# alexxx-db/dbx-distributed-pytorch-examples

Measured on AMD Instinct MI355X. Metric: images/sec (whole node) ResNet-50 ImageNet-1K at 1/2/4/8 MI355X; top-1 acc, higher is better.
Workload: dtype bf16; 1 GPU; model=resnet50 ImageNet-1K 224x224 1000 classes large-batch (global 8192 at 8 GPUs), global_batch=1024, per_gpu_batch=1024, parallelism=dp1, world_size_seen=1, backend=none, impl=native, optimizer=SGD momentum 0.9 nesterov=False wd 5e-5, memory_format=nhwc, graphs=True, ddp=none, kernels=dbx HIP (conv implicit-GEMM MFMA + fused BN/ReLU/pool/CE/SGD)

## Files before the change

### dbx_distributed_pytorch_examples_amd/csrc/nn_ops.hip

```cpp
#include "common.h"
#include "bn_fin.h"
#include "entry.h"

namespace dbx {

__device__ __forceinline__ void shard_sums(const double* stats, int nshard, int C, int c0, double& s_out,
                                           double& q_out, bool& active, int& c) {
  __shared__ double rs[8][33], rq[8][33];
  const int j = threadIdx.x & 7, k = threadIdx.x >> 3;
  c = c0 + j;
  double s = 0.0, q = 0.0;
  if (c < C) {
    for (int kk = k; kk < nshard; kk += 32) { s += stats[(size_t)kk * 2 * C + c]; q += stats[(size_t)kk * 2 * C + C + c]; }
  }
  rs[j][k] = s; rq[j][k] = q;
  __syncthreads();
  active = (k == 0) && (c < C);
  if (active) {
    double ss = 0.0, qq = 0.0;
    for (int t = 0; t < 32; ++t) { ss += rs[j][t]; qq += rq[j][t]; }
    s_out = ss; q_out = qq;
  }
}

// ... 345 lines not shown
    if constexpr (KF > 0) {
      u32x4 win[KF * KF];
      bool ok[KF * KF];
#pragma unroll
      for (int r = 0; r < KF; ++r)
#pragma unroll
        for (int ss = 0; ss < KF; ++ss) {
          const int hh = p * stride - pad + r, w = q * stride - pad + ss;
          const bool v = (unsigned)hh < (unsigned)H && (unsigned)w < (unsigned)W;
          ok[r * KF + ss] = v;
          win[r * KF + ss] = *reinterpret_cast<const u32x4*>(
              x + (((size_t)n * H + (v ? hh : 0)) * W + (v ? w : 0)) * C + c0);
        }
#pragma unroll
      for (int k = 0; k < KF * KF; ++k) {
        float f[8];
        unpack8(win[k], f);
#pragma unroll
        for (int j = 0; j < 8; ++j) {
          float v = f[j] * s[j] + h[j];
          if (relu) v = fmaxf(v, 0.f);
          if (ok[k] && v > best[j]) { best[j] = v; braw[j] = f[j]; bi[j] = (unsigned char)k; }
        }
      }
    }
    for (int r = 0; r < (KF > 0 ? 0 : K); ++r) {
      const int hh = p * stride - pad + r;
      if (hh < 0 || hh >= H) continue;
      for (int ss = 0; ss < K; ++ss) {
        const int w = q * stride - pad + ss;
        if (w < 0 || w >= W) continue;
        float f[8];
        unpack8(*reinterpret_cast<const u32x4*>(x + (((size_t)n * H + hh) * W + w) * C + c0), f);
#pragma unroll
        for (int j = 0; j < 8; ++j) {
          float v = f[j] * s[j] + h[j];
          if (relu) v = fmaxf(v, 0.f);
          if (v > best[j]) { best[j] = v; braw[j] = f[j]; bi[j] = (unsigned char)(r * K + ss); }
        }
      }
    }
    const size_t o = (size_t)pix * C + c0;
    *reinterpret_cast<u32x4*>(out + o) = pack8(best);
    *reinterpret_cast<uint2*>(arg + o) = *reinterpret_cast<uint2*>(bi);
    if (ymax) *reinterpret_cast<u32x4*>(ymax + o) = pack8(braw);
  }
}

__global__ void maxpool_bwd_kernel(const bf16* __restrict__ dout, const unsigned char* __restrict__ arg,
                                   bf16* __restrict__ dx, int N, int H, int W, int C, int P, int Q, int K,
                                   int stride, int pad) {
  const int cpt = C / 8;
  const long long total = (long long)N * H * W * cpt;
  for (long long i = (long long)blockIdx.x * blockDim.x + threadIdx.x; i < total; i += (long long)gridDim.x * blockDim.x) {
    const int cg = (int)(i % cpt);
    long long pix = i / cpt;
    const int w = (int)(pix % W); pix /= W;
    const int h = (int)(pix % H);
    const int n = (int)(pix / H);
    const int c0 = cg * 8;
    float acc[8] = {0, 0, 0, 0, 0, 0, 0, 0};
    const int p_lo = max(0, (h + pad - K + stride) / stride), p_hi = min(P - 1, (h + pad) / stride);
    const int q_lo = max(0, (w + pad - K + stride) / stride), q_hi = min(Q - 1, (w + pad) / stride);
    for (int p = p_lo; p <= p_hi; ++p) {
      const int r = h - (p * stride - pad);
      if (r < 0 || r >= K) continue;
      for (int q = q_lo; q <= q_hi; ++q) {
        const int s = w - (q * stride - pad);
        if (s < 0 || s >= K) continue;
        const size_t o = (((size_t)n * P + p) * Q + q) * C + c0;
        float g[8];
        unpack8(*reinterpret_cast<const u32x4*>(dout + o), g);
        const uint2 av = *reinterpret_cast<const uint2*>(arg + o);
        const unsigned char* a8 = reinterpret_cast<const unsigned char*>(&av);
        const unsigned char me = (unsigned char)(r * K + s);
#pragma unroll
        for (int j = 0; j < 8; ++j) acc[j] += (a8[j] == me) ? g[j] : 0.f;
      }
    }
    *reinterpret_cast<u32x4*>(dx + (((size_t)n * H + h) * W + w) * C + c0) = pack8(acc);
  }
}

template <bool APPLY>
__global__ __launch_bounds__(256) void pool_bn_bwd_kernel(const bf16* __restrict__ dpool,
                                                          const unsigned char* __restrict__ arg,
                                                          const bf16* __restrict__ y, const float* __restrict__ sc,
                                                          const float* __restrict__ sh, const float* __restrict__ c1,
                                                          const float* __restrict__ c2, const float* __restrict__ c3,
                                                          bf16* __restrict__ dy, double* __restrict__ stats, int nshard,
                                                          int N, int H, int W, int C, int P, int Q, int K, int stride,
                                                          int pad) {
  const int cpt = C >> 3;
  const int tid = threadIdx.x;
  const int c0 = (tid % cpt) * 8;
  float s_[8], h_[8], k1[8], k2[8], k3[8];
  load8f(sc + c0, s_);
  load8f(sh + c0, h_);
  load8f(c1 + c0, k1);
  load8f(c2 + c0, k2);
  if (APPLY) load8f(c3 + c0, k3);
  float as[8] = {0, 0, 0, 0, 0, 0, 0, 0}, aq[8] = {0, 0, 0, 0, 0, 0, 0, 0};
  const int rows = N * H, per_row = W * cpt;
  for (int row = blockIdx.x; row < rows; row += gridDim.x) {
    const int n = row / H, h = row - n * H;
    const int p_lo = max(0, (h + pad - K + stride) / stride), p_hi = min(P - 1, (h + pad) / stride);
    const int r_lo = h + pad - p_lo * stride;
    const bool p1 = p_hi >= p_lo, p2 = p_hi > p_lo;
    const int pc = p1 ? p_lo : 0;
    const int prow0 = (n * P + pc) * Q, prow1 = (n * P + (p2 ? p_lo + 1 : pc)) * Q;
    for (int i = tid; i < per_row; i += 256) {
      const int w = i / cpt;
      const int q_lo = max(0, (w + pad - K + stride) / stride);
      u32x4 gd[2][2];
      uint2 av[2][2];
      bool ok[2][2];
#pragma unroll
      for (int t = 0; t < 2; ++t) {
        const int q = q_lo + t;
        const int s = w + pad - q * stride;
        const bool vq = q < Q && s >= 0 && s < K;
        const int qq = vq ? q : 0;
#pragma unroll
        for (int u = 0; u < 2; ++u) {
          const int o = ((u ? prow1 : prow0) + qq) * C + c0;
          gd[u][t] = *reinterpret_cast<const u32x4*>(dpool + o);
          av[u][t] = *reinterpret_cast<const uint2*>(arg + o);
          ok[u][t] = vq && (u == 0 ? p1 : p2);
        }
      }
      const int e = (row * W + w) * C + c0;
      float yv[8];
      unpack8(*reinterpret_cast<const u32x4*>(y + e), yv);
      float g[8] = {0, 0, 0, 0, 0, 0, 0, 0};
#pragma unroll
      for (int u = 0; u < 2; ++u)
#pragma unroll
        for (int t = 0; t < 2; ++t) {
          const int r = r_lo - u * stride, s = w + pad - (q_lo + t) * stride;
          const unsigned me = (unsigned)(r * K + s);
          float gv[8];
          unpack8(gd[u][t], gv);
          const unsigned char* a8 = reinterpret_cast<const unsigned char*>(&av[u][t]);
#pragma unroll
          for (int j = 0; j < 8; ++j) g[j] += (ok[u][t] && a8[j] == me) ? gv[j] : 0.f;
        }
#pragma unroll
      for (int j = 0; j < 8; ++j) g[j] = (yv[j] * s_[j] + h_[j]) > 0.f ? g[j] : 0.f;
      if (APPLY) {
        float o[8];
#pragma unroll
        for (int j = 0; j < 8; ++j) o[j] = k1[j] * g[j] + k2[j] * yv[j] + k3[j];
        *reinterpret_cast<u32x4*>(dy + e) = pack8(o);
      } else {
#pragma unroll
        for (int j = 0; j < 8; ++j) { as[j] += g[j]; aq[j] += g[j] * (yv[j] - k1[j]) * k2[j]; }
      }
    }
  }
  if (!APPLY) {
    __shared__ float red[2][256 * 8];
#pragma unroll
    for (int j = 0; j < 8; ++j) { red[0][tid * 8 + j] = as[j]; red[1][tid * 8 + j] = aq[j]; }
    __syncthreads();
    double* st = stats + (size_t)(blockIdx.x % nshard) * 2 * C;
    for (int c = tid; c < C; c += 256) {
      const int gi = c / 8, j = c % 8;
      float ss = 0.f, qq = 0.f;
      for (int r = 0; r < 256 / cpt; ++r) { ss += red[0][(r * cpt + gi) * 8 + j]; qq += red[1][(r * cpt + gi) * 8 + j]; }
      atomicAdd(st + c, (double)ss);
      atomicAdd(st + C + c, (double)qq);
    }
  }
}

__global__ void avgpool_fwd_kernel(const bf16* __restrict__ x, bf16* __restrict__ out, int N, int HW, int C) {
  const int n = blockIdx.y;
  const int c0 = (blockIdx.x * blockDim.x + threadIdx.x) * 8;
  if (c0 >= C) return;
  float acc[8] = {0, 0, 0, 0, 0, 0, 0, 0};
  for (int i = 0; i < HW; ++i) {
    float f[8];
    unpack8(*reinterpret_cast<const u32x4*>(x + ((size_t)n * HW + i) * C + c0), f);
#pragma unroll
    for (int j = 0; j < 8; ++j) acc[j] += f[j];
  }
  const float inv = 1.f / HW;
#pragma unroll
  for (int j = 0; j < 8; ++j) acc[j] *= inv;
  *reinterpret_cast<u32x4*>(out + (size_t)n * C + c0) = pack8(acc);
}

__global__ void avgpool_bwd_kernel(const bf16* __restrict__ dout, bf16* __restrict__ dx, int N, int HW, int C) {
  const long long total = (long long)N * HW * C / 8;
  const float inv = 1.f / HW;
  for (long long i = (long long)blockIdx.x * blockDim.x + threadIdx.x; i < total; i += (long long)gridDim.x * blockDim.x) {
    const long long e = i * 8;
    const int c0 = (int)(e % C);
    const long long n = e / ((long long)HW * C);
    float f[8];
    unpack8(*reinterpret_cast<const u32x4*>(dout + n * C + c0), f);
#pragma unroll
    for (int j = 0; j < 8; ++j) f[j] *= inv;
    *reinterpret_cast<u32x4*>(dx + e) = pack8(f);
  }
}

template <typename T>
__global__ void softmax_ce_kernel(const T* __restrict__ logits, const long long* __restrict__ labels,
                                  T* __restrict__ dlogits, float* __restrict__ loss_out, double* stats,
                                  int B, int C, float smoothing, float gscale,
                                  const long long* __restrict__ labels2, const float* __restrict__ lam_ptr) {
  const int row = blockIdx.x;
  const T* x = logits + (size_t)row * C;
  const int tid = threadIdx.x;
  __shared__ float red[8];
  __shared__ int redi[8];
  float mx = -INFINITY;
  int amx = 0;
  for (int c = tid; c < C; c += 256) {
    const float v = (float)x[c];
    if (v > mx) { mx = v; amx = c; }
  }
  for (int o = 32; o > 0; o >>= 1) {
    const float om = __shfl_xor(mx, o, 64);
    const int oa = __shfl_xor(amx, o, 64);
    if (om > mx || (om == mx && oa < amx)) { mx = om; amx = oa; }
  }
  const int wid = tid >> 6, lane = tid & 63;
  if (lane == 0) { red[wid] = mx; redi[wid] = amx; }
  __syncthreads();
  if (tid == 0) {
    for (int w = 1; w < 4; ++w)
      if (red[w] > red[0] || (red[w] == red[0] && redi[w] < redi[0])) { red[0] = red[w]; redi[0] = redi[w]; }
  }
  __syncthreads();
  mx = red[0];
  amx = redi[0];
  __syncthreads();
  float se = 0.f, sx = 0.f;
  for (int c = tid; c < C; c += 256) {
    const float v = (float)x[c];
    se += __expf(v - mx);
    sx += v;
// ... 247 lines not shown
extern "C" int dbx_bn_apply(const bf16* y, const float* sc, const float* sh, const bf16* res, const float* rsc,
                            const float* rsh, bf16* out, long long n, int C, int res_mode, int relu,
                            unsigned char* mbits, hipStream_t st, const BnFin* fin, const BnFin* rfin) {
  if (n % C || C % 8 || C / 8 > 256) return -1;
  if (rfin && res_mode != 2) return -2;
  const long long M = n / C;
  const dim3 g(grid_for(M, 256 / (C / 8), (fin || rfin) ? fin_cap(C) : 4096)), b(256);
#define BA(R, A) hipLaunchKernelGGL((bn_apply_kernel<R, A>), g, b, 0, st, y, sc, sh, res, rsc, rsh, out, mbits, M, C, fin, rfin)
  if (res_mode == 0) { if (relu) BA(0, true); else BA(0, false); }
  else if (res_mode == 1) { if (relu) BA(1, true); else BA(1, false); }
  else { if (relu) BA(2, true); else BA(2, false); }
#undef BA
  RET_LAST;
}
extern "C" int dbx_bn_bwd_reduce(const bf16* dout, const bf16* mref, const bf16* y, const float* sc, const float* sh,
                                 const float* mean, const float* invstd, long long M, int C, double* stats,
                                 int nshard, int mask_mode, hipStream_t st) {
  if (C % 8 || C / 8 > 256) return -1;
  const int rpb = 256 / (C / 8);
  const dim3 g(grid_for(M, rpb, 2048)), b(256);
  if (mask_mode == 0) hipLaunchKernelGGL((bn_bwd_reduce_kernel<0>), g, b, 0, st, dout, mref, y, sc, sh, mean, invstd, M, C, stats, nshard);
  else if (mask_mode == 1) hipLaunchKernelGGL((bn_bwd_reduce_kernel<1>), g, b, 0, st, dout, mref, y, sc, sh, mean, invstd, M, C, stats, nshard);
  else hipLaunchKernelGGL((bn_bwd_reduce_kernel<2>), g, b, 0, st, dout, mref, y, sc, sh, mean, invstd, M, C, stats, nshard);
  RET_LAST;
}
extern "C" int dbx_bn_bwd_coeff(const double* stats, int nshard, int C, float count, const float* gamma,
                                const float* mean, const float* invstd, float* coeff, float* dgamma, float* dbeta,
                                int accumulate, hipStream_t st) {
  hipLaunchKernelGGL(bn_bwd_coeff_kernel, dim3((C + 7) / 8), dim3(256), 0, st, stats, nshard, C, count, gamma,
                     mean, invstd, coeff, dgamma, dbeta, accumulate);
  RET_LAST;
}
extern "C" int dbx_bn_bwd_apply(const bf16* dout, const bf16* mref, const bf16* y, const float* sc, const float* sh,
                                const float* coeff, bf16* dy, bf16* gout, long long n, int C, int mask_mode,
                                hipStream_t st, const BnFin* fin) {
  if (n % C || C % 8 || C / 8 > 256) return -1;
  const long long M = n / C;
  const dim3 g(grid_for(M, 256 / (C / 8), fin ? fin_cap(C) : 4096)), b(256);
#define BB(MK, WG) hipLaunchKernelGGL((bn_bwd_apply_kernel<MK, WG>), g, b, 0, st, dout, mref, y, sc, sh, coeff, dy, gout, M, C, fin)
  if (mask_mode == 0) { if (gout) BB(0, true); else BB(0, false); }
  else if (mask_mode == 1) { if (gout) BB(1, true); else BB(1, false); }
  else { if (gout) BB(2, true); else BB(2, false); }
#undef BB
  RET_LAST;
}
extern "C" int dbx_bn_bwd_apply2(const bf16* g, const bf16* y1, const float* c1, bf16* dy1, const bf16* y2,
                                 const float* c2, bf16* dy2, long long n, int C, hipStream_t st, const BnFin* fin1,
                                 const BnFin* fin2) {
  if (n % C || C % 8 || C / 8 > 256) return -1;
  const long long M = n / C;
  hipLaunchKernelGGL(bn_bwd_apply2_kernel, dim3(grid_for(M, 256 / (C / 8), (fin1 || fin2) ? fin_cap(C) : 4096)), dim3(256), 0, st, g, y1, c1, dy1,
                     y2, c2, dy2, M, C, fin1, fin2);
  RET_LAST;
}
extern "C" int dbx_maxpool_fwd(const bf16* x, const float* sc, const float* sh, bf16* out, unsigned char* arg,
                               bf16* ymax, int N, int H, int W, int C, int P, int Q, int K, int stride, int pad, int relu,
                               hipStream_t st, const BnFin* fin) {
  if (C % 8) return -1;
  if (C / 8 > 256) return -1;
  if (fin && !sc) return -2;
  const dim3 grid(grid_for((long long)N * P * Q, 256 / (C / 8), fin ? 1024 : 4096));
  if (K == 3 && (long long)N * P * Q < (1ll << 31))
    hipLaunchKernelGGL(maxpool_fwd_kernel<3>, grid, dim3(256), 0, st, x, sc, sh, out, arg, ymax, N, H, W, C, P, Q, K,
                       stride, pad, relu, fin);
  else
    hipLaunchKernelGGL(maxpool_fwd_kernel<0>, grid, dim3(256), 0, st, x, sc, sh, out, arg, ymax, N, H, W, C, P, Q, K,
                       stride, pad, relu, fin);
  RET_LAST;
}
extern "C" int dbx_maxpool_bwd(const bf16* dout, const unsigned char* arg, bf16* dx, int N, int H, int W, int C, int P,
                               int Q, int K, int stride, int pad, hipStream_t st) {
  if (C % 8) return -1;
  const long long total = (long long)N * H * W * (C / 8);
  hipLaunchKernelGGL(maxpool_bwd_kernel, dim3(grid_for(total)), dim3(256), 0, st, dout, arg, dx, N, H, W, C, P, Q, K,
                     stride, pad);
  RET_LAST;
}
extern "C" int dbx_pool_bn_bwd(const bf16* dpool, const unsigned char* arg, const bf16* y, const float* sc,
                               const float* sh, const float* c1, const float* c2, const float* c3, bf16* dy,
                               double* stats, int nshard, int N, int H, int W, int C, int P, int Q, int K, int stride,
                               int pad, int apply, hipStream_t st) {
  if (C % 8 || 256 % (C / 8) || (K + stride - 1) / stride > 2) return -1;
  if ((long long)N * H * W * C >= (1LL << 31) || (long long)N * P * Q * C >= (1LL << 31)) return -2;
  const dim3 g(grid_for((long long)N * H, 1, apply ? 8192 : 2048)), b(256);
  if (apply)
    hipLaunchKernelGGL((pool_bn_bwd_kernel<true>), g, b, 0, st, dpool, arg, y, sc, sh, c1, c2, c3, dy, stats, nshard,
                       N, H, W, C, P, Q, K, stride, pad);
  else
    hipLaunchKernelGGL((pool_bn_bwd_kernel<false>), g, b, 0, st, dpool, arg, y, sc, sh, c1, c2, c3, dy, stats, nshard,
                       N, H, W, C, P, Q, K, stride, pad);
  RET_LAST;
}
extern "C" int dbx_avgpool_fwd(const bf16* x, bf16* out, int N, int HW, int C, hipStream_t st) {
  if (C % 8) return -1;
  hipLaunchKernelGGL(avgpool_fwd_kernel, dim3((C / 8 + 63) / 64, N), dim3(64), 0, st, x, out, N, HW, C);
  RET_LAST;
}
extern "C" int dbx_avgpool_bwd(const bf16* dout, bf16* dx, int N, int HW, int C, hipStream_t st) {
  if (C % 8) return -1;
  hipLaunchKernelGGL(avgpool_bwd_kernel, dim3(grid_for((long long)N * HW * C / 8)), dim3(256), 0, st, dout, dx, N, HW, C);
  RET_LAST;
}
extern "C" int dbx_softmax_ce(const void* logits, int is_bf16, const long long* labels, void* dlogits, float* loss_out,
                              double* stats, int B, int C, float smoothing, float gscale, const long long* labels2,
                              const float* lam, hipStream_t st, int kind, float target_thresh, int sum_classes) {
  if (kind == 1) {
    if (B <= 0) return 0;
    if (!logits || !labels || C < 1 || (labels2 && !lam)) return -1;
    const dim3 grid((B + 3) / 4);
    if (is_bf16)
      hipLaunchKernelGGL(bce_logits_kernel<bf16>, grid, dim3(256), 0, st, (const bf16*)logits, labels, (bf16*)dlogits,
                         loss_out, stats, B, C, smoothing, gscale, labels2, lam, target_thresh, sum_classes);
    else
      hipLaunchKernelGGL(bce_logits_kernel<float>, grid, dim3(256), 0, st, (const float*)logits, labels,
                         (float*)dlogits, loss_out, stats, B, C, smoothing, gscale, labels2, lam, target_thresh,
                         sum_classes);
    RET_LAST;
  }
  if (kind != 0) return -1;
  if (is_bf16)
    hipLaunchKernelGGL(softmax_ce_kernel<bf16>, dim3(B), dim3(256), 0, st, (const bf16*)logits, labels, (bf16*)dlogits,
                       loss_out, stats, B, C, smoothing, gscale, labels2, lam);
  else
    hipLaunchKernelGGL(softmax_ce_kernel<float>, dim3(B), dim3(256), 0, st, (const float*)logits, labels,
                       (float*)dlogits, loss_out, stats, B, C, smoothing, gscale, labels2, lam);
  RET_LAST;
}
extern "C" int dbx_ce_eval(const void* logits, int is_bf16, const long long* labels, double* stats, int B, int C, int k,
                           const int* nvalid, float* loss_out, int* rank_out, hipStream_t st) {
  if (B <= 0) return 0;
  if (!logits || !labels || !stats || C < 1 || k < 1 || k > C) return -1;
  const dim3 grid((B + 3) / 4);
  if (is_bf16)
    hipLaunchKernelGGL(ce_eval_kernel<bf16>, grid, dim3(256), 0, st, (const bf16*)logits, labels, stats, B, C, k, nvalid,
                       loss_out, rank_out);
  else
    hipLaunchKernelGGL(ce_eval_kernel<float>, grid, dim3(256), 0, st, (const float*)logits, labels, stats, B, C, k,
                       nvalid, loss_out, rank_out);
  RET_LAST;
}
extern "C" int dbx_weight_prep(const float* master, bf16* wbuf, const void* desc_dev, int nlayers, hipStream_t st) {
  hipLaunchKernelGGL(weight_prep_kernel<float>, dim3(512, nlayers), dim3(256), 0, st, master, wbuf,
                     (const WDesc*)desc_dev, nlayers);
  RET_LAST;
}
extern "C" int dbx_weight_prep16(const bf16* src, bf16* wbuf, const void* desc_dev, int nlayers, hipStream_t st) {
  hipLaunchKernelGGL(weight_prep_kernel<bf16>, dim3(512, nlayers), dim3(256), 0, st, src, wbuf,
                     (const WDesc*)desc_dev, nlayers);
  RET_LAST;
}
extern "C" int dbx_cast_f32_bf16(const float* x, bf16* y, long long n, hipStream_t st) {
  hipLaunchKernelGGL(cast_f32_bf16_kernel, dim3(grid_for(n)), dim3(256), 0, st, x, y, n);
  RET_LAST;
}
```

### dbx_distributed_pytorch_examples_amd/engine/program.py

```python
from __future__ import annotations

import math
import os
from dataclasses import dataclass, field
from typing import Dict, List, Optional, Tuple

import torch
import torch.nn as nn

from ..engine_config import EngineConfig
from ..models.resnet import BasicBlock, Bottleneck, CifarBlock, CifarResNet18, ResNet
from ..ops import kernels as K

IMAGENET_MEAN = (0.485, 0.456, 0.406)
IMAGENET_STD = (0.229, 0.224, 0.225)


def _repoint(p: nn.Parameter, view: torch.Tensor) -> None:
    p.data = view
    if p.grad is not None and (p.grad.device != view.device or p.grad.shape != view.shape):
        p.grad = None
    elif p.grad is not None and p.grad.stride() != view.stride():
        g = torch.empty_strided(view.shape, view.stride(), dtype=p.grad.dtype, device=view.device)
        g.copy_(p.grad)
# ... 278 lines not shown
                    _repoint(cv.mod.weight, view)
                    cv.grad = self.grad[off:off + n].view(cv.OC, cv.R * cv.S * cv.IC)
                    self.param_ranges.append((cv.name + ".weight", off, n))
                elif kind in ("bn_w", "bn_b"):
                    bn: BNL = obj
                    mod = bn.mod
                    p = getattr(mod, attr)
                    flat = self.master[off:off + n]
                    flat.copy_(p.detach().to(dev, torch.float32))
                    _repoint(p, flat)
                    if kind == "bn_w":
                        bn.off_w, bn.gamma, bn.dgamma = off, flat, self.grad[off:off + n]
                        bn.gamma_t = flat
                    else:
                        bn.off_b, bn.beta, bn.dbeta = off, flat, self.grad[off:off + n]
                        bn.beta_t = flat
                    self.param_ranges.append((f"{bn.name}.{attr}", off, n))
                    mod.running_mean.data = mod.running_mean.data.to(dev, torch.float32)
                    mod.running_var.data = mod.running_var.data.to(dev, torch.float32)
                    if kind == "bn_w" and mod.num_batches_tracked is not None:
                        nbt_vals.append(int(mod.num_batches_tracked))
                        nbt_mods.append(mod)
                else:
                    p = getattr(self.fc, attr)
                    flat = self.master[off:off + n]
                    flat.copy_(p.detach().reshape(-1).to(dev, torch.float32))
                    view = flat.view(p.shape)
                    _repoint(p, view)
                    if attr == "weight":
                        self.fc_w_off, self.fc_w_grad = off, self.grad[off:off + n].view(p.shape)
                    else:
                        self.fc_b_off, self.fc_b_grad = off, self.grad[off:off + n]
                    self.param_ranges.append((f"fc.{attr}", off, n))
        self.param16 = torch.zeros(total, device=dev, dtype=torch.bfloat16) if self._want_param16 else None
        self.nbt = torch.tensor(nbt_vals, dtype=torch.int64, device=dev)
        for i, mod in enumerate(nbt_mods):
            mod.num_batches_tracked.data = self.nbt[i]
        n16 = 0
        descs = []
        for cv in self.convs:
            if cv.stem:
                continue
            fwd_off = n16
            n16 += cv.numel
            tr_off = n16
            n16 += cv.numel
            descs.append((cv.off, fwd_off, tr_off, cv.OC, cv.R * cv.S, cv.IC))
            cv._w16_off, cv._wt16_off = fwd_off, tr_off
        fc_off = n16
        n16 += self.fc.weight.numel()
        descs.append((self.fc_w_off, fc_off, -1, self.num_classes, 1, self.fc.in_features))
        al = lambda v: (v + 63) // 64 * 64
        st = self.stem
        stem_off = n16 = al(n16)
        n16 += st.OC * 256
        descs.append((st.off, stem_off, -2, st.OC, st.R * 16 + st.S, st.IC))
        fcb_off = n16 = al(n16)
        n16 += self.num_classes
        descs.append((self.fc_b_off, fcb_off, -1, self.num_classes, 1, 1))
        self.w16buf = torch.zeros(al(n16) + 64, device=dev, dtype=torch.bfloat16)
        for cv in self.convs:
            if cv.stem:
                cv.w16 = self.w16buf[stem_off:stem_off + cv.OC * 256].view(cv.OC, 256)
                continue
            cv.w16 = self.w16buf[cv._w16_off:cv._w16_off + cv.numel].view(cv.OC, -1)
            cv.wt16 = self.w16buf[cv._wt16_off:cv._wt16_off + cv.numel].view(cv.IC, -1)
        self.fc_w16 = self.w16buf[fc_off:fc_off + self.fc.weight.numel()].view(self.num_classes, -1)
        self.fc_b16 = self.w16buf[fcb_off:fcb_off + self.num_classes]
        self._wdescs = descs
        self.wdesc = self._pack_wdesc(descs)
        self.n_wdesc = len(descs)
        self.stem_grad_tmp = torch.zeros(self.stem.OC, 256, device=dev, dtype=torch.float32)

    def _alloc_activations(self):
        N, dev, bf = self.N, self.dev, torch.bfloat16
        E = lambda *s: torch.empty(*s, device=dev, dtype=bf)
        st = self.stem
        self.x4 = torch.zeros(N, self.H, self.W, 4, device=dev, dtype=bf)
        self.y0 = E(N, st.OH, st.OW, st.OC)
        ph, pw = self.pool_hw
        self.p0 = E(N, ph, pw, st.OC)
        self.parg = torch.empty(N, ph, pw, st.OC, device=dev, dtype=torch.uint8)
        self.dp0 = E(N, ph, pw, st.OC)
        self.da0 = None if K.pool_bn_bwd_supported(st.OC, self.pool_k, self.pool_s) else E(N, st.OH, st.OW, st.OC)
        self.pymax = E(N, ph, pw, st.OC) if self.da0 is None and self.pool_reduce else None
        self.dy0 = E(N, st.OH, st.OW, st.OC)
        wsmax = 0
        for b in self.blocks:
            b.ys = [E(N, cv.OH, cv.OW, cv.OC) for cv in b.convs]
            b.dys = [E(N, cv.OH, cv.OW, cv.OC) for cv in b.convs]
            b.das = [E(N, cv.OH, cv.OW, cv.OC) for cv in b.convs[:-1]]
            b.acts = [E(N, cv.OH, cv.OW, cv.OC) if self.act_writeback else None for cv in b.convs[:-1]]
            b.mat = [self._materialize(b.convs[j + 1]) and b.acts[j] is not None for j in range(len(b.convs) - 1)]
            h, w, c = b.in_shape
            b.dx = E(N, h, w, c)
            if b.ds_conv is not None:
                dcv = b.ds_conv
                if dcv.R != 1 or dcv.S != 1 or dcv.pad != 0:
                    raise TypeError(f"{dcv.name}: downsample must be a 1x1 pad-0 conv")
                b.yd = E(N, dcv.OH, dcv.OW, dcv.OC)
                b.dyd = E(N, dcv.OH, dcv.OW, dcv.OC)
                b.dsbuf = E(N, dcv.OH, dcv.OW, dcv.IC)
            oh, ow, oc = b.out_shape
            b.out = E(N, oh, ow, oc)
            b.obits = torch.empty(N * oh * ow * oc // 8, device=dev, dtype=torch.uint8)
        for cv in self.convs:
            ktot = 256 if cv.stem else cv.R * cv.S * cv.IC
            wsmax = max(wsmax, cv.OC * ktot)
        self.ws = torch.empty(max(64 * wsmax, 16 << 20), device=dev, dtype=torch.float32)
        fl = self.fwd_flops
        cfg, pol = self.cfg, self.cfg.policy
        self.side_defer = cfg.side_defer if cfg.side_defer is not None else (pol.small(fl) or self.side_block)
        self.side_cu_reserve = (cfg.side_cu_reserve if cfg.side_cu_reserve is not None
                                else (0 if pol.tiny(fl) else 128))
        self.stem_wg_main = cfg.stem_wg_main if cfg.stem_wg_main is not None else (pol.small(fl) or self.side_block)
        self.tail_main = (cfg.tail_main if cfg.tail_main is not None
                          else ((3 if self.side_defer else 2) if pol.mid(fl) else 0))
        self.dwf_cus = cfg.dwf_cus if cfg.dwf_cus is not None else (128 if pol.mid(fl) else 0)
        self.block_tail_main = cfg.block_tail_main
        self._main_tail = []
        self._join_evt = None
        self.event_joins = False
        self.ds_fwd_side = cfg.ds_fwd_side
        self.lazy_join = cfg.lazy_join if cfg.lazy_join is not None else (pol.tiny(fl) or self.side_block)
        self._pending_side = []
        self.ws_stem = (torch.empty(40 << 20, device=dev, dtype=torch.float32)
                        if dev.type == "cuda" and self.stem_wg_main else self.ws)
        self.ws_main = (torch.empty_like(self.ws) if ((self.tail_main > 0 or self.block_tail_main > 0)
                                                      and dev.type == "cuda"
                                                       and self.overlap_wgrad) else self.ws)
        fused = [b.convs[-1] for i, b in enumerate(self.blocks) if self._fuse3(b, i == len(self.blocks) - 1)]
        self.ws_dw = (torch.empty((max((K.dwfused_grid(c.IC, c.OC) + 64) * c.OC * c.IC for c in fused)
                                   if dev.type == "cuda" else 16), device=dev, dtype=torch.float32)
                      if fused else None)
        fh, fw = self.feat_hw
        self.dfeat = self.blocks[-1].out
        self.dlast = E(N, fh, fw, self.feat_c)
        self.g_last = E(N, fh, fw, self.feat_c)
        self.pooled = E(N, self.feat_c)
        self.dpooled = E(N, self.feat_c)
        self.logits = E(N, self.num_classes)
        self.dlogits = E(N, self.num_classes)
        self.head_ws = (torch.empty(8 * max(N * self.num_classes, self.num_classes * self.feat_c), device=dev,
                                    dtype=torch.float32) if dev.type == "cuda" else None)
        self.labels = torch.zeros(N, device=dev, dtype=torch.int64)
        sh, sw = self.src_hw
        self.src_ch = 3 if self.in_ch != 1 else 1
        self.src_tab = None
        if self.src_ragged is None:
            self.img_u8 = torch.zeros(N, sh, sw, self.src_ch, device=dev, dtype=torch.uint8)
            self.boxes = torch.tensor([[0.0, 0.0, float(sh), float(sw)]] * N, device=dev)
        else:
            self.img_u8 = torch.zeros(N * sh * ((sw * self.src_ch + 15) // 16 * 16), device=dev, dtype=torch.uint8)
            self.src_tab = torch.tensor([[0, 1, 1, 16]] * N, device=dev, dtype=torch.int32)
            self.boxes = torch.tensor([[0.0, 0.0, 1.0, 1.0]] * N, device=dev)
        self.flip = torch.zeros(N, device=dev, dtype=torch.uint8)
        self.metrics = torch.zeros(2, device=dev, dtype=torch.float64)
        ns = self.nshard
        self.stats_region = torch.zeros(sum(2 * 2 * ns * bn.C for bn in self.bns), device=dev, dtype=torch.float64)
        o = 0
        for bn in self.bns:
            bn.stats = self.stats_region[o:o + 2 * ns * bn.C]
            o += 2 * ns * bn.C
            bn.bstats = self.stats_region[o:o + 2 * ns * bn.C]
            o += 2 * ns * bn.C
        self.bn_arena = torch.zeros(sum(7 * bn.C for bn in self.bns), device=dev, dtype=torch.float32)
        o = 0
# ... 606 lines not shown
                            in_scale=pbn.scale, in_shift=pbn.shift, relu_in=True)
            if kw is not None:
                K.conv_dgrad(src, cv.wt16, b.das[j - 1], R=cv.R, S=cv.S, stride=cv.stride, pad=cv.pad,
                             epilogue=K.BNBwdEpilogue(K.MASK_Y, b.ys[j - 1], pbn.mean, pbn.invstd, pbn.bstats,
                                                      scale=pbn.scale, shift=pbn.shift,
                                                      act_out=None if b.mat[j - 1] else act,
                                                      fin1=pbn.fin_b if self._fused_fin(pbn) else None), **kw)
            if act is not None:
                self._wgrad(b.dys[j], act, cv.grad, self.ws, R=cv.R, S=cv.S, stride=cv.stride, pad=cv.pad)
            elif kw and not pre:
                self._wgrad(b.dys[j], b.ys[j - 1], cv.grad, self.ws, R=cv.R, S=cv.S, stride=cv.stride, pad=cv.pad,
                            in_scale=pbn.scale, in_shift=pbn.shift, relu_in=True)
            pcount = N * pc.OH * pc.OW
            fold = self._fold(pc)
            fin = None
            if kw is None or not self._fused_fin(pbn):
                if not fold and self._cin(pbn, pcount):
                    fin = pbn.fin_b
                else:
                    self._coeff(pbn, pcount)
            if fold:
                pend = dict(bwd_y=b.ys[j - 1], bwd_coeff=pbn.coeff, dy_out=b.dys[j - 1])
                gin = b.das[j - 1]
            else:
                K.bn_bwd_apply(b.das[j - 1], b.ys[j - 1], pbn.coeff, b.dys[j - 1], mask_mode=K.MASK_NONE, fin=fin)
        c0 = b.convs[0]
        kw0, src0 = (pend, gin) if pend else ({}, b.dys[0])
        if not kw0:
            self._wgrad(b.dys[0], x, c0.grad, self.ws, R=c0.R, S=c0.S, stride=c0.stride, pad=c0.pad)
        if b.ds_conv is not None:
            dc = b.ds_conv
            if ds_fold is None:
                self._wgrad(b.dyd, x, dc.grad, self.ws, R=dc.R, S=dc.S, stride=dc.stride, pad=dc.pad)
                K.conv_dgrad(b.dyd, dc.wt16, b.dsbuf, R=1, S=1, stride=1, pad=0)
            else:
                K.conv_dgrad(g, dc.wt16, b.dsbuf, R=1, S=1, stride=1, pad=0, **ds_fold)
                self._wgrad(b.dyd, x, dc.grad, self.ws, R=dc.R, S=dc.S, stride=dc.stride, pad=dc.pad)
            addsrc, sub = b.dsbuf, dc.stride
        else:
            addsrc, sub = g, 1
        epi = None
        if i > 0:
            pb = self.blocks[i - 1]
            epi = K.BNBwdEpilogue(K.MASK_OUT, pb.ys[-1], pb.bns[-1].mean, pb.bns[-1].invstd, pb.bns[-1].bstats,
                                  mbits=pb.obits,
                                  ybn2=pb.yd if pb.ds_conv is not None else None,
                                  mean2=pb.ds_bn.mean if pb.ds_conv is not None else None,
                                  inv2=pb.ds_bn.invstd if pb.ds_conv is not None else None,
                                  stats2=pb.ds_bn.bstats if pb.ds_conv is not None else None,
                                  fin1=pb.bns[-1].fin_b if self._fused_fin(pb.bns[-1]) else None,
                                  fin2=(pb.ds_bn.fin_b if pb.ds_conv is not None and self._fused_fin(pb.ds_bn)
                                        else None))
        K.conv_dgrad(src0, c0.wt16, b.dx, R=c0.R, S=c0.S, stride=c0.stride, pad=c0.pad,
                     addsrc=addsrc, add_sub=sub, epilogue=epi, **kw0)
        if kw0:
            self._wgrad(b.dys[0], x, c0.grad, self.ws, R=c0.R, S=c0.S, stride=c0.stride, pad=c0.pad)

    def fwd_conv_flops(self) -> float:
        return sum(2.0 * self.N * cv.OH * cv.OW * cv.OC * cv.R * cv.S * cv.IC for cv in self.convs)

    def _materialize(self, cv: ConvL) -> bool:
        if not (self.fast_mat and self.dev.type == "cuda" and cv.stride == 1
                and cv.R == 3):
            return False
        t = K.pick_tile(self.N * cv.OH * cv.OW, cv.OC, "fwd0", cv.IC, cv.R, cv.stride)
        return len(t) > 2 and t[2] in (4, 5)

    def _fuse3(self, b: BlockL, last: bool) -> bool:
        if not self.fuse_dw or last or b.kind != "bottleneck":
            return False
        c3 = b.convs[-1]
        return ((c3.R, c3.S, c3.stride, c3.pad) == (1, 1, 1, 0) and c3.OH >= self.cfg.fuse_dw_min_hw
                and K.dwfused_preferred(c3.IC, c3.OC, self.N * c3.OH * c3.OW))

    def _fold(self, cv, dense: bool = False) -> bool:
        stride = 1 if dense else cv.stride
        return (self.fuse_bwd_apply and not cv.stem and self.N * cv.OH * cv.OW * cv.OC >= self.fold_min
                and (cv.IC <= self.fold_max_ratio * cv.OC or cv.OH >= self.fold_ratio_min_hw)
                and K.tail_supported(cv.OC, cv.R, cv.S, stride, cv.pad))

    def _bwd_stem(self):
        st, sbn = self.stem, self.stem_bn
        dp = self.blocks[0].dx
        if K.pool_bn_bwd_supported(st.OC, self.pool_k, self.pool_s):
            pk = dict(K=self.pool_k, stride=self.pool_s, pad=self.pool_p)
            if self.pymax is not None:
                K.bn_bwd_reduce(dp, self.pymax, sbn.mean, sbn.invstd, sbn.bstats, mask_mode=K.MASK_Y,
                                scale=sbn.scale, shift=sbn.shift)
            else:
                K.pool_bn_bwd_reduce(dp, self.parg, self.y0, sbn.scale, sbn.shift, sbn.mean, sbn.invstd, sbn.bstats,
                                     **pk)
            K.bn_bwd_coeff(sbn.bstats, self.N * st.OH * st.OW, sbn.gamma, sbn.mean, sbn.invstd, sbn.coeff,
                           sbn.dgamma, sbn.dbeta)
            if self.fuse_stem_bwd and K.stem_bwd_supported(st.OC, self.pool_k, self.pool_s, st.R, st.S):
                K.stem_bwd_fused(dp, self.parg, self.y0, sbn.scale, sbn.shift, sbn.coeff, self.x4, self.stem_grad_tmp,
                                 self.ws, R=st.R, S=st.S, conv_stride=st.stride, conv_pad=st.pad, **pk)
                g = self.grad[st.off:st.off + st.numel].view(st.OC, st.R, st.S, st.IC)
                g.copy_(self.stem_grad_tmp.view(st.OC, 8, 8, 4)[:, :st.R, :st.S, :st.IC])
                return
            K.pool_bn_bwd_apply(dp, self.parg, self.y0, sbn.scale, sbn.shift, sbn.coeff, self.dy0, **pk)
        else:
            K.maxpool_bwd(dp, self.parg, self.da0, K=self.pool_k, stride=self.pool_s, pad=self.pool_p)
            self._bn_bwd(sbn, self.da0, self.y0, self.dy0, self.N * st.OH * st.OW, K.MASK_Y)
        on_main = ((self.side_batch or self.side_block) and self.dev.type == "cuda" and self.overlap_wgrad
                   and self.stem_wg_main)

        def stem_wgrad():
            g = self.grad[st.off:st.off + st.numel]
            out = K.conv_wgrad(self.dy0, self.x4, self.stem_grad_tmp, self.ws_stem if on_main else self.ws, R=st.R,
                               S=st.S, stride=st.stride, pad=st.pad, stem=True, out_krsc=g)
            if out is not g:
                g.view(st.OC, st.R, st.S, st.IC).copy_(self.stem_grad_tmp.view(st.OC, 8, 8, 4)[:, :st.R, :st.S, :st.IC])
        if on_main:
            stem_wgrad()
        else:
            self._side(stem_wgrad)

    def backward(self):
        for _, fn in self._segments:
            fn()

    def segment_param_ranges(self) -> List[List[Tuple[str, int, int]]]:
        groups = []
        by_prefix = {"head": ["fc."], "layer4": ["layer4."], "layer3": ["layer3."], "layer2": ["layer2."],
                     "layer1": ["layer1."], "stem": ["conv1.", "bn1."]}
        for name, _ in self._segments:
            pre = by_prefix[name]
            groups.append([r for r in self.param_ranges if any(r[0].startswith(p) for p in pre)])
        return groups
```

### dbx_distributed_pytorch_examples_amd/ops/kernels.py

```python
from __future__ import annotations

import os
from typing import Optional, Tuple

import torch

from ..utils import debug as _debug
from . import reference as _ref
from ._ext import C, stream_ptr, use_native
from ..engine_config import EngineConfig

_E = EngineConfig.current

FWD, DGRAD, STEM, FWD_PATCH, DGRAD_PATCH = 0, 1, 2, 3, 4
_SPLITK = ("ksplit", "kper", "skws", "skcnt")
MASK_NONE, MASK_OUT, MASK_Y = 0, 1, 2


_POST_LAUNCH = None


def set_post_launch(cb, owner=None) -> None:
    global _POST_LAUNCH
    if cb is None and owner is not None and _POST_LAUNCH is not None and _POST_LAUNCH != owner:
# ... 849 lines not shown
    _ref.check_channels(Cc)
    _chk(dout, torch.bfloat16, "dout", y.numel())
    _chk(y, torch.bfloat16, "y")
    nsh = _chk_stats(stats, "stats", Cc)
    if mask_mode == MASK_OUT:
        _chk(mref, torch.bfloat16, "mref", y.numel())
    C().bn_bwd_reduce(dout.data_ptr(), _p(mref), y.data_ptr(), _p(scale), _p(shift), mean.data_ptr(),
                      invstd.data_ptr(), y.numel() // Cc, Cc, stats.data_ptr(), nsh, mask_mode, stream_ptr())


@_dispatch
def bn_bwd_coeff(stats, count, gamma, mean, invstd, coeff, dgamma=None, dbeta=None, accumulate=False):
    Cc = mean.numel()
    C().bn_bwd_coeff(stats.data_ptr(), _nsh(stats, Cc), Cc, float(count), _p(gamma), mean.data_ptr(), invstd.data_ptr(),
                     coeff.data_ptr(), _p(dgamma), _p(dbeta), int(accumulate), stream_ptr())


@_dispatch
def bn_bwd_apply(dout, y, coeff, dy, *, mask_mode, mref=None, scale=None, shift=None, gout=None, fin=None):
    Cc = y.shape[-1]
    _ref.check_channels(Cc)
    _chk(dy, torch.bfloat16, "dy", y.numel())
    if gout is not None:
        _chk(gout, torch.bfloat16, "gout", y.numel())
    if fin is not None and fin.desc is None:
        fin.run()
        fin = None
    C().bn_bwd_apply(dout.data_ptr(), _p(mref), y.data_ptr(), _p(scale), _p(shift), coeff.data_ptr(),
                     dy.data_ptr(), _p(gout), y.numel(), Cc, mask_mode, stream_ptr(), fin.ptr() if fin else 0)


@_dispatch
def bn_bwd_apply2(g, y1, coeff1, dy1, y2, coeff2, dy2, fin1=None, fin2=None):
    Cc = y1.shape[-1]
    _ref.check_channels(Cc)
    for t, nm in ((g, "g"), (y1, "y1"), (dy1, "dy1"), (y2, "y2"), (dy2, "dy2")):
        _chk(t, torch.bfloat16, nm, y1.numel())
    _chk(coeff1, torch.float32, "coeff1", 3 * Cc)
    _chk(coeff2, torch.float32, "coeff2", 3 * Cc)
    fins = []
    for f in (fin1, fin2):
        if f is not None and f.desc is None:
            f.run()
            f = None
        fins.append(f.ptr() if f else 0)
    C().bn_bwd_apply2(g.data_ptr(), y1.data_ptr(), coeff1.data_ptr(), dy1.data_ptr(), y2.data_ptr(),
                      coeff2.data_ptr(), dy2.data_ptr(), y1.numel(), Cc, stream_ptr(), *fins)


@_dispatch
def maxpool_fwd(x, out, arg, *, K=3, stride=2, pad=1, scale=None, shift=None, relu=True, ymax=None, fin=None):
    N, H, W, Cc = x.shape
    _, P, Q, _ = out.shape
    _ref.check_channels(Cc)
    _chk(x, torch.bfloat16, "x")
    _chk(out, torch.bfloat16, "out")
    _chk(arg, torch.uint8, "arg", out.numel())
    if ymax is not None:
        _chk(ymax, torch.bfloat16, "ymax", out.numel())
    if fin is not None and (fin.desc is None or scale is None):
        fin.run()
        fin = None
    C().maxpool_fwd(x.data_ptr(), _p(scale), _p(shift), out.data_ptr(), arg.data_ptr(), _p(ymax), N, H, W, Cc, P, Q,
                    K, stride, pad, int(relu), stream_ptr(), fin.ptr() if fin else 0)


@_dispatch
def maxpool_bwd(dout, arg, dx, *, K=3, stride=2, pad=1):
    N, H, W, Cc = dx.shape
    _, P, Q, _ = dout.shape
    _chk(dout, torch.bfloat16, "dout")
    _chk(arg, torch.uint8, "arg", dout.numel())
    _chk(dx, torch.bfloat16, "dx")
    C().maxpool_bwd(dout.data_ptr(), arg.data_ptr(), dx.data_ptr(), N, H, W, Cc, P, Q, K, stride, pad, stream_ptr())


def _pool_bn_bwd_check(dpool, arg, y, K, stride):
    N, H, W, Cc = y.shape
    _chk(dpool, torch.bfloat16, "dpool")
    _chk(arg, torch.uint8, "arg", dpool.numel())
    _chk(y, torch.bfloat16, "y")
    if dpool.shape[0] != N or dpool.shape[3] != Cc:
        raise ValueError("pool_bn_bwd: dpool / y shapes disagree")
    if Cc % 8 or 256 % (Cc // 8) or (K + stride - 1) // stride > 2:
        raise ValueError("pool_bn_bwd: unsupported channel count / pool geometry")
    return N, H, W, Cc, dpool.shape[1], dpool.shape[2]


def pool_bn_bwd_supported(C: int, K: int, stride: int) -> bool:
    return C % 8 == 0 and 256 % (C // 8) == 0 and (K + stride - 1) // stride <= 2


@_dispatch
def pool_bn_bwd_reduce(dpool, arg, y, scale, shift, mean, invstd, stats, *, K=3, stride=2, pad=1):
    N, H, W, Cc, Pp, Q = _pool_bn_bwd_check(dpool, arg, y, K, stride)
    nsh = _chk_stats(stats, "stats", Cc)
    C().pool_bn_bwd(dpool.data_ptr(), arg.data_ptr(), y.data_ptr(), scale.data_ptr(), shift.data_ptr(),
                    mean.data_ptr(), invstd.data_ptr(), 0, 0, stats.data_ptr(), nsh, N, H, W, Cc, Pp, Q, K,
                    stride, pad, 0, stream_ptr())


@_dispatch
def pool_bn_bwd_apply(dpool, arg, y, scale, shift, coeff, dy, *, K=3, stride=2, pad=1):
    N, H, W, Cc, Pp, Q = _pool_bn_bwd_check(dpool, arg, y, K, stride)
    _chk(dy, torch.bfloat16, "dy", y.numel())
    C().pool_bn_bwd(dpool.data_ptr(), arg.data_ptr(), y.data_ptr(), scale.data_ptr(), shift.data_ptr(),
                    coeff.data_ptr(), coeff.data_ptr() + 4 * Cc, coeff.data_ptr() + 8 * Cc, dy.data_ptr(), 0, 1,
                    N, H, W, Cc, Pp, Q, K, stride, pad, 1, stream_ptr())


def stem_bwd_supported(C: int, K: int, stride: int, R: int, S: int) -> bool:
    return C == 64 and R <= 8 and S <= 8 and (K + stride - 1) // stride <= 2


@_dispatch
def stem_bwd_fused(dpool, arg, y, scale, shift, coeff, x4, dw, ws, *, K=3, stride=2, pad=1, R=7, S=7,
                   conv_stride=2, conv_pad=3):
    N, H, W, Cc, Pp, Q = _pool_bn_bwd_check(dpool, arg, y, K, stride)
    _chk(x4, torch.bfloat16, "x4")
    _chk(coeff, torch.float32, "coeff", 3 * Cc)
    _chk(scale, torch.float32, "scale", Cc)
    _chk(shift, torch.float32, "shift", Cc)
    _chk(dw, torch.float32, "dw", Cc * 256)
    _chk(ws, torch.float32, "ws")
    Nx, IH, IW, C4 = x4.shape
    if Nx != N or C4 != 4 or conv_out_hw(IH, IW, R, S, conv_stride, conv_pad) != (H, W):
        raise ValueError("stem_bwd_fused: image / stem output shapes disagree")
    if not stem_bwd_supported(Cc, K, stride, R, S):
        raise ValueError("stem_bwd_fused: unsupported geometry")
    n = C().stem_bwd(dpool=dpool.data_ptr(), arg=arg.data_ptr(), y=y.data_ptr(), sc=scale.data_ptr(),
                     sh=shift.data_ptr(), coeff=coeff.data_ptr(), x4=x4.data_ptr(), ws=ws.data_ptr(), ws_cap=ws.numel(),
                     N=N, H=H, W=W, C=Cc, P=Pp, Q=Q, PK=K, pstride=stride, ppad=pad, IH=IH, IW=IW, R=R, S=S,
                     stride=conv_stride, pad=conv_pad, fused=1, st=stream_ptr())
    C().wgrad_reduce(ws.data_ptr(), dw.data_ptr(), Cc * 256, n, 1.0, 0, stream_ptr())
    return dw


@_dispatch
def avgpool_fwd(x, out):
    N, H, W, Cc = x.shape
    _chk(x, torch.bfloat16, "x")
    _chk(out, torch.bfloat16, "out", N * Cc)
    C().avgpool_fwd(x.data_ptr(), out.data_ptr(), N, H * W, Cc, stream_ptr())


@_dispatch
def avgpool_bwd(dout, dx):
    N, H, W, Cc = dx.shape
    _chk(dout, torch.bfloat16, "dout", N * Cc)
    _chk(dx, torch.bfloat16, "dx")
    C().avgpool_bwd(dout.data_ptr(), dx.data_ptr(), N, H * W, Cc, stream_ptr())


@_dispatch
def softmax_ce(logits, labels, dlogits=None, loss_out=None, stats=None, smoothing=0.0, grad_scale=1.0,
               labels2=None, lam=None):
    B, Cc = logits.shape
    if logits.dtype not in (torch.float32, torch.bfloat16) or not logits.is_contiguous():
        raise TypeError("logits must be contiguous fp32/bf16")
    _chk(labels, torch.int64, "labels", B)
    if dlogits is not None:
        _chk(dlogits, logits.dtype, "dlogits", B * Cc)
    if stats is not None:
        _chk(stats, torch.float64, "stats", 2)
    if (labels2 is None) != (lam is None):
        raise ValueError("labels2 and lam come together")
    if labels2 is not None:
        _chk(labels2, torch.int64, "labels2", B)
        _chk(lam, torch.float32, "lam", 1)
    C().softmax_ce(logits.data_ptr(), int(logits.dtype == torch.bfloat16), labels.data_ptr(), _p(dlogits),
                   _p(loss_out), _p(stats), B, Cc, float(smoothing), float(grad_scale), _p(labels2), _p(lam),
                   stream_ptr(), 0, -1.0, 0)

# ... 553 lines not shown
```

Baseline: 17050 images/s.

## Stage pooled grad and argmax bands in LDS for stem pool+BN backward

Reworks the fused maxpool/BN backward kernel so each block handles a band of input rows and first copies the needed pooled-gradient and argmax rows into dynamic shared memory. The overlapping pool windows then read from LDS instead of re-reading global memory for every input row. The y loads are also batched with ILP=4. Band height is picked to fit an LDS budget, and a support check on pooled width is added. The cost is large dynamic LDS, which lowers occupancy, plus extra syncthreads per band.

```diff
diff --git a/dbx_distributed_pytorch_examples_amd/csrc/nn_ops.hip b/dbx_distributed_pytorch_examples_amd/csrc/nn_ops.hip
--- a/dbx_distributed_pytorch_examples_amd/csrc/nn_ops.hip
+++ b/dbx_distributed_pytorch_examples_amd/csrc/nn_ops.hip
@@ -451,6 +451,7 @@
   }
 }
 
+constexpr int PB_ILP = 4;
 template <bool APPLY>
 __global__ __launch_bounds__(256) void pool_bn_bwd_kernel(const bf16* __restrict__ dpool,
                                                           const unsigned char* __restrict__ arg,
@@ -459,7 +460,11 @@
                                                           const float* __restrict__ c2, const float* __restrict__ c3,
                                                           bf16* __restrict__ dy, double* __restrict__ stats, int nshard,
                                                           int N, int H, int W, int C, int P, int Q, int K, int stride,
-                                                          int pad) {
+                                                          int pad, int BH, int PR) {
+  extern __shared__ __attribute__((aligned(16))) unsigned char pb_lds[];
+  const int rowe = Q * C;
+  bf16* sg = reinterpret_cast<bf16*>(pb_lds);
+  unsigned char* sa = pb_lds + (size_t)PR * rowe * sizeof(bf16);
   const int cpt = C >> 3;
   const int tid = threadIdx.x;
   const int c0 = (tid % cpt) * 8;
@@ -470,65 +475,93 @@
   load8f(c2 + c0, k2);
   if (APPLY) load8f(c3 + c0, k3);
   float as[8] = {0, 0, 0, 0, 0, 0, 0, 0}, aq[8] = {0, 0, 0, 0, 0, 0, 0, 0};
-  const int rows = N * H, per_row = W * cpt;
-  for (int row = blockIdx.x; row < rows; row += gridDim.x) {
-    const int n = row / H, h = row - n * H;
-    const int p_lo = max(0, (h + pad - K + stride) / stride), p_hi = min(P - 1, (h + pad) / stride);
-    const int r_lo = h + pad - p_lo * stride;
-    const bool p1 = p_hi >= p_lo, p2 = p_hi > p_lo;
-    const int pc = p1 ? p_lo : 0;
-    const int prow0 = (n * P + pc) * Q, prow1 = (n * P + (p2 ? p_lo + 1 : pc)) * Q;
-    for (int i = tid; i < per_row; i += 256) {
-      const int w = i / cpt;
-      const int q_lo = max(0, (w + pad - K + stride) / stride);
-      u32x4 gd[2][2];
-      uint2 av[2][2];
-      bool ok[2][2];
-#pragma unroll
-      for (int t = 0; t < 2; ++t) {
-        const int q = q_lo + t;
-        const int s = w + pad - q * stride;
-        const bool vq = q < Q && s >= 0 && s < K;
-        const int qq = vq ? q : 0;
-#pragma unroll
-        for (int u = 0; u < 2; ++u) {
-          const int o = ((u ? prow1 : prow0) + qq) * C + c0;
-          gd[u][t] = *reinterpret_cast<const u32x4*>(dpool + o);
-          av[u][t] = *reinterpret_cast<const uint2*>(arg + o);
-          ok[u][t] = vq && (u == 0 ? p1 : p2);
+  const int per_row = W * cpt;
+  const int bpi = (H + BH - 1) / BH, nbands = N * bpi;
+  for (int band = blockIdx.x; band < nbands; band += gridDim.x) {
+    const int n = band / bpi, h0 = (band - n * bpi) * BH, h1 = min(H, h0 + BH);
+    const int pb = max(0, (h0 + pad - K + stride) / stride), pe = min(P - 1, (h1 - 1 + pad) / stride);
+    const int nel = min(max(pe - pb + 1, 0), PR) * rowe, src = (n * P + pb) * rowe;
+    for (int i = tid * 8; i < nel; i += 256 * 8)
+      *reinterpret_cast<u32x4*>(sg + i) = *reinterpret_cast<const u32x4*>(dpool + src + i);
+    if ((rowe & 15) == 0) {
+      for (int i = tid * 16; i < nel; i += 256 * 16)
+        *reinterpret_cast<u32x4*>(sa + i) = *reinterpret_cast<const u32x4*>(arg + src + i);
+    } else {
+      for (int i = tid * 8; i < nel; i += 256 * 8)
+        *reinterpret_cast<uint2*>(sa + i) = *reinterpret_cast<const uint2*>(arg + src + i);
+    }
+    __syncthreads();
+    for (int h = h0; h < h1; ++h) {
+      const int row = n * H + h;
+      const int p_lo = max(0, (h + pad - K + stride) / stride), p_hi = min(P - 1, (h + pad) / stride);
+      const int r_lo = h + pad - p_lo * stride;
+      const bool p1 = p_hi >= p_lo, p2 = p_hi > p_lo;
+      const int pc = p1 ? p_lo - pb : 0;
+      const int prow0 = pc * Q, prow1 = (p2 ? pc + 1 : pc) * Q;
+      for (int i0 = tid; i0 < per_row; i0 += 256 * PB_ILP) {
+        u32x4 yr[PB_ILP];
+#pragma unroll
+        for (int k = 0; k < PB_ILP; ++k) {
+          const int i = i0 + 256 * k;
+          if (i < per_row) yr[k] = *reinterpret_cast<const u32x4*>(y + (row * W + i / cpt) * C + c0);
+        }
+#pragma unroll
+        for (int k = 0; k < PB_ILP; ++k) {
+          const int i = i0 + 256 * k;
+          if (i >= per_row) break;
+          const int w = i / cpt;
+          const int q_lo = max(0, (w + pad - K + stride) / stride);
+          u32x4 gd[2][2];
+          uint2 av[2][2];
+          bool ok[2][2];
+#pragma unroll
+          for (int t = 0; t < 2; ++t) {
+            const int q = q_lo + t;
+            const int s = w + pad - q * stride;
+            const bool vq = q < Q && s >= 0 && s < K;
+            const int qq = vq ? q : 0;
+#pragma unroll
+            for (int u = 0; u < 2; ++u) {
+              const int o = ((u ? prow1 : prow0) + qq) * C + c0;
+              gd[u][t] = *reinterpret_cast<const u32x4*>(sg + o);
+              av[u][t] = *reinterpret_cast<const uint2*>(sa + o);
+              ok[u][t] = vq && (u == 0 ? p1 : p2);
+            }
+          }
+          const int e = (row * W + w) * C + c0;
+          float yv[8];
+          unpack8(yr[k], yv);
+          float g[8] = {0, 0, 0, 0, 0, 0, 0, 0};
+#pragma unroll
+          for (int u = 0; u < 2; ++u)
+#pragma unroll
+            for (int t = 0; t < 2; ++t) {
+              const int r = r_lo - u * stride, s = w + pad - (q_lo + t) * stride;
+              const unsigned me = (unsigned)(r * K + s);
+              float gv[8];
+              unpack8(gd[u][t], gv);
+              const unsigned char* a8 = reinterpret_cast<const unsigned char*>(&av[u][t]);
+#pragma unroll
+              for (int j = 0; j < 8; ++j) g[j] += (ok[u][t] && a8[j] == me) ? gv[j] : 0.f;
+            }
+#pragma unroll
+          for (int j = 0; j < 8; ++j) g[j] = (yv[j] * s_[j] + h_[j]) > 0.f ? g[j] : 0.f;
+          if (APPLY) {
+            float o[8];
+#pragma unroll
+            for (int j = 0; j < 8; ++j) o[j] = k1[j] * g[j] + k2[j] * yv[j] + k3[j];
+            *reinterpret_cast<u32x4*>(dy + e) = pack8(o);
+          } else {
+#pragma unroll
+            for (int j = 0; j < 8; ++j) { as[j] += g[j]; aq[j] += g[j] * (yv[j] - k1[j]) * k2[j]; }
+          }
         }
       }
-      const int e = (row * W + w) * C + c0;
-      float yv[8];
-      unpack8(*reinterpret_cast<const u32x4*>(y + e), yv);
-      float g[8] = {0, 0, 0, 0, 0, 0, 0, 0};
-#pragma unroll
-      for (int u = 0; u < 2; ++u)
-#pragma unroll
-        for (int t = 0; t < 2; ++t) {
-          const int r = r_lo - u * stride, s = w + pad - (q_lo + t) * stride;
-          const unsigned me = (unsigned)(r * K + s);
-          float gv[8];
-          unpack8(gd[u][t], gv);
-          const unsigned char* a8 = reinterpret_cast<const unsigned char*>(&av[u][t]);
-#pragma unroll
-          for (int j = 0; j < 8; ++j) g[j] += (ok[u][t] && a8[j] == me) ? gv[j] : 0.f;
-        }
-#pragma unroll
-      for (int j = 0; j < 8; ++j) g[j] = (yv[j] * s_[j] + h_[j]) > 0.f ? g[j] : 0.f;
-      if (APPLY) {
-        float o[8];
-#pragma unroll
-        for (int j = 0; j < 8; ++j) o[j] = k1[j] * g[j] + k2[j] * yv[j] + k3[j];
-        *reinterpret_cast<u32x4*>(dy + e) = pack8(o);
-      } else {
-#pragma unroll
-        for (int j = 0; j < 8; ++j) { as[j] += g[j]; aq[j] += g[j] * (yv[j] - k1[j]) * k2[j]; }
-      }
-    }
+    }
+    __syncthreads();
   }
   if (!APPLY) {
-    __shared__ float red[2][256 * 8];
+    float(*red)[256 * 8] = reinterpret_cast<float(*)[256 * 8]>(pb_lds);
 #pragma unroll
     for (int j = 0; j < 8; ++j) { red[0][tid * 8 + j] = as[j]; red[1][tid * 8 + j] = aq[j]; }
     __syncthreads();
@@ -942,13 +975,23 @@
                                int pad, int apply, hipStream_t st) {
   if (C % 8 || 256 % (C / 8) || (K + stride - 1) / stride > 2) return -1;
   if ((long long)N * H * W * C >= (1LL << 31) || (long long)N * P * Q * C >= (1LL << 31)) return -2;
-  const dim3 g(grid_for((long long)N * H, 1, apply ? 8192 : 2048)), b(256);
+  constexpr long long kBandLds = 40 * 1024, kMaxLds = 64 * 1024;
+  int BH = 4, PR = 0;
+  long long lds = 0;
+  for (;; BH >>= 1) {
+    PR = (BH + K - 2) / stride + 1;
+    lds = 3ll * PR * Q * C;
+    if (lds <= kBandLds || BH == 1) break;
+  }
+  if (lds > kMaxLds) return -3;
+  if (!apply && lds < 2 * 256 * 8 * (long long)sizeof(float)) lds = 2 * 256 * 8 * sizeof(float);
+  const dim3 g(grid_for((long long)N * ((H + BH - 1) / BH), 1, apply ? (1 << 20) : 2048)), b(256);
   if (apply)
-    hipLaunchKernelGGL((pool_bn_bwd_kernel<true>), g, b, 0, st, dpool, arg, y, sc, sh, c1, c2, c3, dy, stats, nshard,
-                       N, H, W, C, P, Q, K, stride, pad);
+    hipLaunchKernelGGL((pool_bn_bwd_kernel<true>), g, b, (size_t)lds, st, dpool, arg, y, sc, sh, c1, c2, c3, dy, stats,
+                       nshard, N, H, W, C, P, Q, K, stride, pad, BH, PR);
   else
-    hipLaunchKernelGGL((pool_bn_bwd_kernel<false>), g, b, 0, st, dpool, arg, y, sc, sh, c1, c2, c3, dy, stats, nshard,
-                       N, H, W, C, P, Q, K, stride, pad);
+    hipLaunchKernelGGL((pool_bn_bwd_kernel<false>), g, b, (size_t)lds, st, dpool, arg, y, sc, sh, c1, c2, c3, dy, stats,
+                       nshard, N, H, W, C, P, Q, K, stride, pad, BH, PR);
   RET_LAST;
 }
 extern "C" int dbx_avgpool_fwd(const bf16* x, bf16* out, int N, int HW, int C, hipStream_t st) {
diff --git a/dbx_distributed_pytorch_examples_amd/engine/program.py b/dbx_distributed_pytorch_examples_amd/engine/program.py
--- a/dbx_distributed_pytorch_examples_amd/engine/program.py
+++ b/dbx_distributed_pytorch_examples_amd/engine/program.py
@@ -384,7 +384,7 @@
         self.p0 = E(N, ph, pw, st.OC)
         self.parg = torch.empty(N, ph, pw, st.OC, device=dev, dtype=torch.uint8)
         self.dp0 = E(N, ph, pw, st.OC)
-        self.da0 = None if K.pool_bn_bwd_supported(st.OC, self.pool_k, self.pool_s) else E(N, st.OH, st.OW, st.OC)
+        self.da0 = None if K.pool_bn_bwd_supported(st.OC, self.pool_k, self.pool_s, pw) else E(N, st.OH, st.OW, st.OC)
         self.pymax = E(N, ph, pw, st.OC) if self.da0 is None and self.pool_reduce else None
         self.dy0 = E(N, st.OH, st.OW, st.OC)
         wsmax = 0
@@ -1157,7 +1157,7 @@
     def _bwd_stem(self):
         st, sbn = self.stem, self.stem_bn
         dp = self.blocks[0].dx
-        if K.pool_bn_bwd_supported(st.OC, self.pool_k, self.pool_s):
+        if self.da0 is None:
             pk = dict(K=self.pool_k, stride=self.pool_s, pad=self.pool_p)
             if self.pymax is not None:
                 K.bn_bwd_reduce(dp, self.pymax, sbn.mean, sbn.invstd, sbn.bstats, mask_mode=K.MASK_Y,
diff --git a/dbx_distributed_pytorch_examples_amd/ops/kernels.py b/dbx_distributed_pytorch_examples_amd/ops/kernels.py
--- a/dbx_distributed_pytorch_examples_amd/ops/kernels.py
+++ b/dbx_distributed_pytorch_examples_amd/ops/kernels.py
@@ -955,13 +955,14 @@
     _chk(y, torch.bfloat16, "y")
     if dpool.shape[0] != N or dpool.shape[3] != Cc:
         raise ValueError("pool_bn_bwd: dpool / y shapes disagree")
-    if Cc % 8 or 256 % (Cc // 8) or (K + stride - 1) // stride > 2:
-        raise ValueError("pool_bn_bwd: unsupported channel count / pool geometry")
+    if not pool_bn_bwd_supported(Cc, K, stride, dpool.shape[2]):
+        raise ValueError("pool_bn_bwd: unsupported channel count / pool geometry / pooled width")
     return N, H, W, Cc, dpool.shape[1], dpool.shape[2]
 
 
-def pool_bn_bwd_supported(C: int, K: int, stride: int) -> bool:
-    return C % 8 == 0 and 256 % (C // 8) == 0 and (K + stride - 1) // stride <= 2
+def pool_bn_bwd_supported(C: int, K: int, stride: int, Q: int = 0) -> bool:
+    return (C % 8 == 0 and 256 % (C // 8) == 0 and (K + stride - 1) // stride <= 2
+            and 3 * ((K - 1) // stride + 1) * Q * C <= 64 * 1024)
 
 
 @_dispatch
```

Measured after the change: 16940 images/s. No clear change (-0.6%).
